# torognes/vsearch

Hardware: AMD Instinct MI355X
Metric: GCUPS (useful DP cells/s of the search16 global-alignment path: DP + traceback + CIGAR) (higher is better)
Workload: dtype int16

## Files before the change

include/vsx.h:

```cpp
#ifndef VSX_H
#define VSX_H

#include <stddef.h>
#include <stdint.h>

#ifdef __cplusplus
extern "C" {
#endif

#define VSX_API_VERSION 1000
#define VSX_SCORE_SENTINEL 32767

#define VSX_OK         0
#define VSX_EINVAL    -1
#define VSX_ENODEVICE -2
#define VSX_ENOMEM    -3
#define VSX_EHIP      -4

typedef struct vsx_ctx vsx_ctx;
typedef struct vsx_seqset vsx_seqset;
typedef struct vsx_plan vsx_plan;

typedef struct vsx_scoring {
  int64_t match;
  int64_t mismatch;
  int64_t gap_open_query_left;
  int64_t gap_open_target_left;
  int64_t gap_open_query_interior;
  int64_t gap_open_target_interior;
  int64_t gap_open_query_right;
  int64_t gap_open_target_right;
  int64_t gap_ext_query_left;
  int64_t gap_ext_target_left;
  int64_t gap_ext_query_interior;
  int64_t gap_ext_target_interior;
  int64_t gap_ext_query_right;
  int64_t gap_ext_target_right;
  int32_t n_mismatch;
} vsx_scoring;

typedef struct vsx_results {
  uint64_t   n_pairs;
  int16_t  * score;
  uint16_t * aligned;
  uint16_t * matches;
  uint16_t * mismatches;
  uint16_t * gaps;
  uint64_t * cigar_off;
  char     * cigar_blob;
  uint64_t   cigar_bytes;
  uint8_t  * verdict;
} vsx_results;

#define VSX_VERDICT_UNDECIDED 0
#define VSX_VERDICT_ACCEPTED  1
#define VSX_VERDICT_WEAK      2
#define VSX_VERDICT_REJECTED  3
typedef struct vsx_filter {
  int32_t iddef;
  int32_t leftjust, rightjust;
  int32_t pad;
  double  id, weak_id, maxid, mid, query_cov, target_cov;
  int64_t maxsubs, maxgaps, mincols, maxdiffs;
} vsx_filter;
int vsx_plan_set_filter(vsx_plan * plan, const vsx_filter * f);

typedef struct vsx_timing {
  float    forward_ms;
  float    traceback_ms;
  float    total_ms;
  uint32_t forward_launches;
  uint32_t traceback_launches;
  uint64_t cells;
  uint64_t dir_bytes;
} vsx_timing;

typedef struct vsx_plan_info {
  uint64_t tasks;
  uint64_t tasks_tilted;
  uint64_t tasks_tracked;
  uint32_t rows_dominant;
  uint32_t chunks;
  uint64_t tasks_max3;
  uint64_t tasks_sparse;
  uint64_t waves;
  uint64_t tasks_pair;
  uint64_t tasks_split;
} vsx_plan_info;

const char * vsx_version_string(void);
int vsx_device_count(void);
const char * vsx_last_error(void);

int vsx_create(vsx_ctx ** out, const vsx_scoring * scoring, int device);
void vsx_destroy(vsx_ctx * ctx);


int vsx_seqset_create(vsx_ctx * ctx, vsx_seqset ** out, uint64_t n,
                      const char * blob, uint64_t blob_bytes,
                      const uint64_t * offsets, const uint32_t * lengths);
int vsx_seqset_create_from_device(vsx_ctx * ctx, vsx_seqset ** out, uint64_t n,
                                  const void * d_blob, uint64_t blob_bytes,
                                  const uint64_t * offsets, const uint32_t * lengths);
int vsx_seqset_create_both_strands(vsx_ctx * ctx, vsx_seqset ** out, uint64_t n,
                                   const char * blob, uint64_t blob_bytes,
                                   const uint64_t * offsets, const uint32_t * lengths);
void vsx_seqset_destroy(vsx_seqset * s);
uint64_t vsx_seqset_count(const vsx_seqset * s);

int vsx_plan_create(vsx_ctx * ctx, vsx_plan ** out,
                    const vsx_seqset * queries, const vsx_seqset * targets,
                    uint64_t n_pairs, const uint32_t * qidx, const uint32_t * tidx,
                    uint64_t dir_budget_bytes);
int vsx_plan_run(vsx_plan * plan);
int vsx_plan_sync(vsx_plan * plan, vsx_timing * timing );
int vsx_plan_fetch(vsx_plan * plan, vsx_results * out);
int vsx_plan_describe(const vsx_plan * plan, vsx_plan_info * info);
#define VSX_HIT_RECORD_BYTES 24
int vsx_plan_export_hits(vsx_plan * plan, void * d_dst, uint64_t dst_bytes);
int vsx_plan_export_runs(vsx_plan * plan, void * d_dst, uint64_t dst_bytes, uint64_t * n_runs);
int64_t vsx_cigar_from_runs(const uint32_t * runs, uint32_t n, char * dst, uint64_t cap);
void vsx_plan_destroy(vsx_plan * plan);

int vsx_align_pairs_filtered(vsx_ctx * ctx, const vsx_seqset * queries, const vsx_seqset * targets,
                             uint64_t n_pairs, const uint32_t * qidx, const uint32_t * tidx,
                             const vsx_filter * filter, vsx_results * out);
int vsx_align_pairs(vsx_ctx * ctx, const vsx_seqset * queries, const vsx_seqset * targets,
// ... 27 lines not shown
```

vsearch_amd/_lib.py:

```python
import ctypes as C
import os

HERE = os.path.dirname(os.path.abspath(__file__))
LIB_PATH = os.environ.get("VSX_LIBRARY") or os.path.join(HERE, "libvsx.so")

VSX_OK, VSX_EINVAL, VSX_ENODEVICE, VSX_ENOMEM, VSX_EHIP = 0, -1, -2, -3, -4
SENTINEL = 32767

SYMBOLS = [
    "vsx_version_string", "vsx_device_count", "vsx_last_error", "vsx_create", "vsx_destroy",
    "vsx_seqset_create", "vsx_seqset_create_both_strands", "vsx_seqset_create_from_device", "vsx_seqset_destroy", "vsx_seqset_count",
    "vsx_plan_create", "vsx_plan_run", "vsx_plan_sync", "vsx_plan_fetch", "vsx_plan_export_hits", "vsx_plan_export_runs",
    "vsx_cigar_from_runs", "vsx_plan_destroy",
    "vsx_align_pairs", "vsx_align_pairs_filtered", "vsx_align_pairs_ranked", "vsx_ranked_free", "vsx_plan_set_filter", "vsx_results_free", "vsx_plan_describe",
]
EXACT_SYMBOLS = ["vsx_search_exact", "vsx_search_exact_last_stats", "vsx_internal_search_exact_host"]
SEARCH_SYMBOLS = ["vsx_search_opts_default", "vsx_searcher_create", "vsx_searcher_destroy", "vsx_searcher_db_text", "vsx_search_batch",
                  "vsx_search_batch_meta", "vsx_searcher_set_meta",
                  "vsx_hits_free", "vsx_search_candidates", "vsx_search_candidates_batch", "vsx_candidates_free", "vsx_lma_align", "vsx_allpairs_block", "vsx_allpairs_rows", "vsx_allpairs_stream", "vsx_cluster_fast", "vsx_cluster_out_free", "vsx_msa", "vsx_msa_out_free",
                  "vsx_msa_device", "vsx_msa_device_batch", "vsx_dust_mask", "vsx_abundance_ratio_cmp",
                  "vsx_multi_searcher_create", "vsx_multi_searcher_destroy", "vsx_multi_searcher_devices", "vsx_multi_searcher_replica",
                  "vsx_multi_search_batch", "vsx_multi_allpairs",
                  "vsx_chimera_opts_default", "vsx_uchime_ref", "vsx_chimera_last_stats",
                  "vsx_chimera_denovo_opts_default", "vsx_uchime_denovo", "vsx_chimera_denovo_last_stats",
# ... 294 lines not shown
class OrientResult(C.Structure):
    _fields_ = [("n_queries", C.c_uint64), ("n_fwd", C.c_uint64), ("n_rev", C.c_uint64), ("n_none", C.c_uint64),
                ("rec", C.POINTER(OrientRecord)), ("text", C.c_void_p), ("qual", C.c_void_p)]


class OrientStats(C.Structure):
    _fields_ = [(n, C.c_uint64) for n in ("queries_device", "queries_host_wordlength", "queries_host_qlen", "queries_host_forced")] + \
               [("queries_class", C.c_uint64 * ORIENT_CLASSES)] + \
               [(n, C.c_uint64) for n in ("windows", "words_distinct", "build_chunks", "build_keys")] + \
               [(n, C.c_double) for n in ("seconds_build", "seconds_stage", "seconds_count", "seconds_emit", "seconds_output",
                                          "seconds_total")]


class Scoring(C.Structure):
    _fields_ = [(n, C.c_int64) for n in (
        "match", "mismatch", "gap_open_query_left", "gap_open_target_left", "gap_open_query_interior",
        "gap_open_target_interior", "gap_open_query_right", "gap_open_target_right",
        "gap_ext_query_left", "gap_ext_target_left", "gap_ext_query_interior", "gap_ext_target_interior",
        "gap_ext_query_right", "gap_ext_target_right")] + [("n_mismatch", C.c_int32)]


class Results(C.Structure):
    _fields_ = [("n_pairs", C.c_uint64), ("score", C.POINTER(C.c_int16)), ("aligned", C.POINTER(C.c_uint16)),
                ("matches", C.POINTER(C.c_uint16)), ("mismatches", C.POINTER(C.c_uint16)),
                ("gaps", C.POINTER(C.c_uint16)), ("cigar_off", C.POINTER(C.c_uint64)),
                ("cigar_blob", C.POINTER(C.c_char)), ("cigar_bytes", C.c_uint64), ("verdict", C.POINTER(C.c_uint8))]


class Ranked(C.Structure):
    _fields_ = [("n_pairs", C.c_uint64), ("n_hits", C.c_uint64), ("pair", C.POINTER(C.c_uint32)), ("score", C.POINTER(C.c_int16)),
                ("aligned", C.POINTER(C.c_uint16)), ("matches", C.POINTER(C.c_uint16)), ("mismatches", C.POINTER(C.c_uint16)),
                ("gaps", C.POINTER(C.c_uint16)), ("verdict", C.POINTER(C.c_uint8)), ("id", C.POINTER(C.c_double)),
                ("cigar_off", C.POINTER(C.c_uint64)), ("cigar_blob", C.POINTER(C.c_char)), ("cigar_bytes", C.c_uint64),
                ("n_undecided", C.c_uint64), ("undecided", C.POINTER(C.c_uint32))]


class Filter(C.Structure):
    _fields_ = [("iddef", C.c_int32), ("leftjust", C.c_int32), ("rightjust", C.c_int32), ("pad", C.c_int32),
                ("id", C.c_double), ("weak_id", C.c_double), ("maxid", C.c_double), ("mid", C.c_double),
                ("query_cov", C.c_double), ("target_cov", C.c_double),
                ("maxsubs", C.c_int64), ("maxgaps", C.c_int64), ("mincols", C.c_int64), ("maxdiffs", C.c_int64)]


class PlanInfo(C.Structure):
    _fields_ = [("tasks", C.c_uint64), ("tasks_tilted", C.c_uint64), ("tasks_tracked", C.c_uint64),
                ("rows_dominant", C.c_uint32), ("chunks", C.c_uint32), ("tasks_max3", C.c_uint64),
                ("tasks_sparse", C.c_uint64), ("waves", C.c_uint64), ("tasks_pair", C.c_uint64),
                ("tasks_split", C.c_uint64)]


class Timing(C.Structure):
    _fields_ = [("forward_ms", C.c_float), ("traceback_ms", C.c_float), ("total_ms", C.c_float),
                ("forward_launches", C.c_uint32), ("traceback_launches", C.c_uint32),
                ("cells", C.c_uint64), ("dir_bytes", C.c_uint64)]


class ClusterOut(C.Structure):
    _fields_ = [("n", C.c_uint64), ("n_clusters", C.c_uint64), ("clusterno", C.POINTER(C.c_uint32)), ("hits", Hits)]


class MsaOut(C.Structure):
    _fields_ = [("alnlen", C.c_uint64), ("n_rows", C.c_uint64), ("conslen", C.c_uint64), ("rows", C.POINTER(C.c_char)),
                ("consensus", C.POINTER(C.c_char)), ("profile", C.POINTER(C.c_uint64))]


_lib = None


def load():
    global _lib
    if _lib is not None:
        return _lib
    if not os.path.exists(LIB_PATH):
        raise ImportError(
            f"{LIB_PATH} not found: build the HIP extension first (python -c 'import __graft_entry__ as g; "
            "g.build()' or make -C vsearch_amd/csrc). vsearch_amd has no CPU fallback.")
    lib = C.CDLL(LIB_PATH)
    vp = C.c_void_p
    lib.vsx_version_string.restype = C.c_char_p
    lib.vsx_last_error.restype = C.c_char_p
    lib.vsx_device_count.restype = C.c_int
    lib.vsx_create.argtypes = [C.POINTER(vp), C.POINTER(Scoring), C.c_int]
    lib.vsx_destroy.argtypes = [vp]
    lib.vsx_destroy.restype = None
    lib.vsx_seqset_create.argtypes = [vp, C.POINTER(vp), C.c_uint64, vp, C.c_uint64, vp, vp]
    lib.vsx_seqset_create_both_strands.argtypes = [vp, C.POINTER(vp), C.c_uint64, vp, C.c_uint64, vp, vp]
    lib.vsx_seqset_create_from_device.argtypes = [vp, C.POINTER(vp), C.c_uint64, vp, C.c_uint64, vp, vp]
    lib.vsx_seqset_destroy.argtypes = [vp]
    lib.vsx_seqset_destroy.restype = None
    lib.vsx_seqset_count.argtypes = [vp]
    lib.vsx_seqset_count.restype = C.c_uint64
    lib.vsx_plan_create.argtypes = [vp, C.POINTER(vp), vp, vp, C.c_uint64, vp, vp, C.c_uint64]
    lib.vsx_plan_run.argtypes = [vp]
    lib.vsx_plan_sync.argtypes = [vp, C.POINTER(Timing)]
    lib.vsx_plan_fetch.argtypes = [vp, C.POINTER(Results)]
    lib.vsx_plan_export_hits.argtypes = [vp, vp, C.c_uint64]
    lib.vsx_plan_export_runs.argtypes = [vp, vp, C.c_uint64, C.POINTER(C.c_uint64)]
    lib.vsx_cigar_from_runs.argtypes = [vp, C.c_uint32, vp, C.c_uint64]
    lib.vsx_cigar_from_runs.restype = C.c_int64
    lib.vsx_plan_destroy.argtypes = [vp]
    lib.vsx_plan_destroy.restype = None
    lib.vsx_plan_describe.argtypes = [vp, C.POINTER(PlanInfo)]
    lib.vsx_internal_settle_counts.argtypes = [vp, C.POINTER(C.c_uint64 * 2)]
    lib.vsx_internal_export_host.argtypes = [vp, vp, vp, C.c_uint64, C.POINTER(C.c_uint64)]
    lib.vsx_align_pairs.argtypes = [vp, vp, vp, C.c_uint64, vp, vp, C.POINTER(Results)]
    lib.vsx_align_pairs_filtered.argtypes = [vp, vp, vp, C.c_uint64, vp, vp, C.POINTER(Filter), C.POINTER(Results)]
    lib.vsx_align_pairs_ranked.argtypes = [vp, vp, vp, C.c_uint64, vp, vp, C.POINTER(Filter), C.c_int, C.POINTER(Ranked)]
# ... 140 lines not shown
```

vsearch_amd/csrc/vsx_device.hip:

```cpp
#include <hip/hip_runtime.h>
#include <type_traits>
#include <cstdlib>
#include <atomic>
#include "vsx_internal.h"

typedef unsigned int u32;
typedef unsigned int u32x4 __attribute__((ext_vector_type(4)));
typedef unsigned int u32x3 __attribute__((ext_vector_type(3)));
typedef short s2 __attribute__((ext_vector_type(2)));
typedef unsigned short us2 __attribute__((ext_vector_type(2)));

#define DEV __device__ __forceinline__
struct __attribute__((aligned(4))) Pair2 { unsigned int x, y; };

#define SIGN2 0x80008000u

DEV s2 S2(u32 x) { return __builtin_bit_cast(s2, x); }
DEV us2 U2(u32 x) { return __builtin_bit_cast(us2, x); }
DEV u32 UI(s2 x) { return __builtin_bit_cast(u32, x); }
DEV u32 UI(us2 x) { return __builtin_bit_cast(u32, x); }

DEV u32 sadd(u32 a, u32 b) { return UI(__builtin_elementwise_add_sat(S2(a), S2(b))); }
DEV u32 ssub(u32 a, u32 b) { return UI(__builtin_elementwise_sub_sat(S2(a), S2(b))); }
DEV u32 pmax(u32 a, u32 b) { return UI(__builtin_elementwise_max(S2(a), S2(b))); }
// ... 582 lines not shown
                  constexpr int NF = R + (R + 1) / 2;
                  constexpr int NFH = RT + (RT + 1) / 2, ZH = 4 * VSX_COLCK_NBH(RT);
                  auto flatc = [&](int z) -> u32 {
                    if (MIDCK)
                      {
                        const int hh = z / ZH, zz = z % ZH, r00 = hh * RT;
                        if (zz < RT) return hout[r00 + zz] + CK_REBIAS;
                        if (zz < NFH)
                          {
                            const int r0 = r00 + 2 * (zz - RT), r1 = (r0 + 1 < r00 + RT) ? r0 + 1 : r0;
                            return __builtin_amdgcn_perm(psubw(hout[r1], E[r1]), psubw(hout[r0], E[r0]), 0x06040200u);
                          }
                        return 0u;
                      }
                    if (z < R) return hout[z] + CK_REBIAS;
                    if (z < NF)
                      {
                        const int r0 = 2 * (z - R), r1 = r0 + 1 < R ? r0 + 1 : r0;
                        return __builtin_amdgcn_perm(psubw(hout[r1], E[r1]), psubw(hout[r0], E[r0]), 0x06040200u);
                      }
                    return 0u;
                  };
#pragma unroll
                  for (int z = 0; z < 4 * VSX_COLCK_NB(R, true); z += 4)
                    __builtin_nontemporal_store((u32x4) {flatc(z), flatc(z + 1), flatc(z + 2), flatc(z + 3)}, reinterpret_cast<u32x4 *>(cb + VSX_COLCK_CDW(VSX_COLCK_NB(R, true), ck_slot, z >> 2)));
                }
              else if (R % 2 == 0)
                {
                  auto flat = [&](int z) -> u32 { return z < R ? hout[z] : E[z - R]; };
#pragma unroll
                  for (int z = 0; z < 2 * R; z += 4)
                    __builtin_nontemporal_store((u32x4) {flat(z), flat(z + 1), flat(z + 2), flat(z + 3)}, reinterpret_cast<u32x4 *>(cb + VSX_COLCK_DW(R, lane, z >> 2)));
                }
              else
                {
                  u32 * cp = cb + lane * (2 * R);
#pragma unroll
                  for (int x = 0; x < R; ++x) { cp[x] = hout[x]; cp[R + x] = E[x]; }
                }
            }
          if (QPL) sym = symn;
      };
      int t_switch = 0;
      if (P.share_sub)
        {
          int dmin = 0x7fffffff;
          if (DA > 0 && DA < dmin) dmin = DA;
          if (DB > 0 && DB < dmin) dmin = DB;
#pragma unroll
          for (int m = 32; m >= 1; m >>= 1) { const int o = __shfl_xor(dmin, m, 64); dmin = o < dmin ? o : dmin; }
          t_switch = __builtin_amdgcn_readfirstlane(dmin == 0x7fffffff ? 0 : dmin - 1) & ~1;
          if (t_switch > steps) t_switch = steps & ~1;
        }
      int t = 0;
      qrt = qrt_i_pk; rt = pack16(P.rt_i);
      for (; t < t_switch && (TRACK || t < 16); t += 2)
        {
          step(t, hprev, hnext, profA, profB, std::true_type {}, std::false_type {}, std::false_type {});
          step(t + 1, hnext, hprev, profB, profA, std::true_type {}, std::true_type {}, std::false_type {});
        }
      if (!TRACK)
        {
          const u32 lpk = (u32) l * 0x00010001u;
          lv1 = psubw(lv1, psubw(0u, lpk));
          for (; t + 32 <= t_switch; t += 16)
            {
              const int tb = t & ~15;
#pragma unroll
              for (int k = 0; k < 16; k += 2)
                {
                  step(tb + k, hprev, hnext, profA, profB, std::true_type {}, std::false_type {}, std::integral_constant<int, 2> {});
                  step(tb + k + 1, hnext, hprev, profB, profA, std::true_type {}, std::true_type {}, std::integral_constant<int, 2> {});
                }
            }
          for (; t < t_switch; t += 2)
            {
              step(t, hprev, hnext, profA, profB, std::true_type {}, std::false_type {}, std::true_type {});
              step(t + 1, hnext, hprev, profB, profA, std::true_type {}, std::true_type {}, std::true_type {});
            }
          lv1 = psubw(lv1, lpk);
        }
      for (; t < steps; t += 2)
        {
          step(t, hprev, hnext, profA, profB, std::false_type {}, std::false_type {}, std::false_type {});
          step(t + 1, hnext, hprev, profB, profA, std::false_type {}, std::true_type {}, std::false_type {});
        }

      if (s + 1 < nstrips)
        {
          __builtin_amdgcn_fence(__ATOMIC_RELEASE, "agent");
          __builtin_amdgcn_fence(__ATOMIC_ACQUIRE, "agent");
        }
    }

#pragma unroll
  for (int m = 8; m >= 1; m >>= 1)
    {
      hmin = pmin(hmin, (u32) __shfl_xor((int) hmin, m, 16));
      hmax = pmax(hmax, (u32) __shfl_xor((int) hmax, m, 16));
    }
  const int l_last = (total_lanes - 1) & 15;
  score = (u32) __shfl((int) score, l_last, 16);
  leave = (u32) __shfl((int) leave, l_last, 16);
  if (l == 0)
    {
      const int mnA = (int16_t) (hmin & 0xffff), mnB = (int16_t) (hmin >> 16);
      const int mxA = (int16_t) (hmax & 0xffff), mxB = (int16_t) (hmax >> 16);
      VsxSlotOut oA, oB;
      score = psubw(score, BIAS);
      oA.score = (int16_t) ((int) (int16_t) (score & 0xffff) - (DA > 0 ? (Q + DA - 2) * tl : 0));
      oB.score = (int16_t) ((int) (int16_t) (score >> 16) - (DB > 0 ? (Q + DB - 2) * tl : 0));
      oA.leave = (uint16_t) (leave & 0xffff); oB.leave = (uint16_t) (leave >> 16); oA.pad = 0; oB.pad = 0;
      oA.overflow = (mnA <= P.smin || mxA >= 32767) ? 1 : 0;
      oB.overflow = (mnB <= P.smin || mxB >= 32767) ? 1 : 0;
      if (sub_on)
        {
          slot_out[(size_t) tix * VSX_TASK_SLOTS + 2 * g] = oA;
          slot_out[(size_t) tix * VSX_TASK_SLOTS + 2 * g + 1] = oB;
        }
    }
}

DEV u32 half_lo(u32 w, bool hi) { return hi ? (w >> 16) : w; }
DEV int wave_max_i32(int v)
{
#pragma unroll
  for (int m = 32; m >= 1; m >>= 1) { const int o = __shfl_xor(v, m, 64); v = o > v ? o : v; }
  return v;
}

DEV void rank_note(const VsxFilterDev & FL, u32 pid, u32 verdict, int score, double idv)
{
  if (FL.rank_counts == nullptr) return;
// ... 1340 lines not shown
```

vsearch_amd/csrc/vsx_host.cpp:

```cpp
#include "../../include/vsx.h"
#include "vsx_internal.h"
#include "vsx_private.h"

#include <hip/hip_runtime.h>
#include <algorithm>
#include <cinttypes>
#include <cstdio>
#include <cstdlib>
#include <cstring>
#include <sched.h>
#include <thread>
#include <atomic>
#include <condition_variable>
#include <mutex>
#include <chrono>
#include <deque>
#include <functional>
#include <memory>
#include <numeric>
#include <string>
#include <vector>

using vsxp::fail;
using vsxp::DevBuf;
// ... 616 lines not shown
          vsx_launch_max3_selftest(d_bad.p, c->stream) == hipSuccess &&
          hipMemcpyAsync(bad2, d_bad.p, 8, hipMemcpyDeviceToHost, c->stream) == hipSuccess && hipStreamSynchronize(c->stream) == hipSuccess)
        {
          const uint32_t bad = bad2[0];
          if (bad) std::fprintf(stderr, "libvsx: device %d: v_pk_maximum3_f16 disagrees with the integer maximum on %u probes -- MAX3 class disabled\n", device, bad);
          g_max3_state[device].store(bad ? 2 : 1);
          if (bad2[1])
            {
              std::fprintf(stderr, "libvsx: device %d: v_perm_b32 sign selectors disagree on %u probes -- the first traceback kernel is used\n", device, bad2[1]);
              vsx_internal_set_tb_v2(device, 0);
            }
        }
      else
        {
          (void) hipGetLastError();
          std::fprintf(stderr, "libvsx: device %d: the MAX3 / v_perm_b32 self-test could not run -- MAX3 class and second traceback kernel disabled\n", device);
          g_max3_state[device].store(2);
          vsx_internal_set_tb_v2(device, 0);
        }
    }
  else if (device >= 64) vsx_internal_set_tb_v2(device, 0);

  if (geqi == geti && geti > 0 && P.share_sub && !c->tb_packed && !c->force_fallback &&
      std::min(match, mism) + 2 * geti >= 0 && 2 * geti - geql >= 0 &&
      std::max(match, mism) + 2 * geti <= 255 && 2 * geti - geql <= 255 &&
      geti <= 127 && std::max({goqi, goti, goqr + geqr - geti, gotr + getr - geti, goql + geql + goqi}) <= 127 &&
      !(std::getenv("VSX_TILT") && std::strcmp(std::getenv("VSX_TILT"), "0") == 0))
    {
      const int g = geti;
      VsxDevParams & T = c->Pt;
      T = P;
      T.tilt = g;
      T.qrq_i_pk = pk(goqi + geqi - g); T.rq_i_pk = pk(geqi - g);
      T.qrq_r_pk = pk(goqr + geqr - g); T.rq_r_pk = pk(geqr - g);
      T.qrt_i = goti + geti - g; T.rt_i = geti - g;
      T.qrt_r = gotr + getr - g; T.rt_r = getr - g;
      std::vector<int16_t> htop_t(VSX_TABLE_LEN), hleft_t(VSX_TABLE_LEN), matrix_t(256);
      for (int j = 0; j < VSX_TABLE_LEN; ++j)
        {
          htop_t[j] = (int16_t) sat16((int) htop[j] + (j - 1) * g);
          hleft_t[j] = (int16_t) sat16((int) hleft[j] + (j - 1) * g);
        }
      for (int x = 0; x < 256; ++x) matrix_t[x] = (int16_t) sat16(matrix[x] + 2 * g);
      if ((e = c->d_htop_t.alloc(VSX_TABLE_LEN)) != hipSuccess || (e = c->d_hleft_t.alloc(VSX_TABLE_LEN)) != hipSuccess ||
          (e = c->d_matrix_t.alloc(256)) != hipSuccess ||
          (e = hipMemcpy(c->d_htop_t.p, htop_t.data(), VSX_TABLE_LEN * 2, hipMemcpyHostToDevice)) != hipSuccess ||
          (e = hipMemcpy(c->d_hleft_t.p, hleft_t.data(), VSX_TABLE_LEN * 2, hipMemcpyHostToDevice)) != hipSuccess ||
          (e = hipMemcpy(c->d_matrix_t.p, matrix_t.data(), 512, hipMemcpyHostToDevice)) != hipSuccess)
        {
          cleanup();
          return fail(VSX_EHIP, "vsx_create: %s", hipGetErrorString(e));
        }
      T.htop = c->d_htop_t.p; T.hleft = c->d_hleft_t.p; T.matrix = c->d_matrix_t.p;
    }
  { std::lock_guard<std::mutex> lk(g_ctx_mu); g_ctxs.push_back(c); }
  *out = c;
  return VSX_OK;
}

void vsx_destroy(vsx_ctx * c)
{
  if (!c) return;
  { std::lock_guard<std::mutex> lk(g_ctx_mu); g_ctxs.erase(std::remove(g_ctxs.begin(), g_ctxs.end(), c), g_ctxs.end()); }
  (void) hipSetDevice(c->device);
  if (c->stream) { (void) hipStreamSynchronize(c->stream); (void) hipStreamDestroy(c->stream); }
  if (c->stream2) { (void) hipStreamSynchronize(c->stream2); (void) hipStreamDestroy(c->stream2); }
  if (c->stream_b) { (void) hipStreamSynchronize(c->stream_b); (void) hipStreamDestroy(c->stream_b); }
  if (c->stream_up) { (void) hipStreamSynchronize(c->stream_up); (void) hipStreamDestroy(c->stream_up); }
  if (c->stream_dn) { (void) hipStreamSynchronize(c->stream_dn); (void) hipStreamDestroy(c->stream_dn); }
  c->shared_dir[0].reset();
  c->shared_dir[1].reset();
  c->shared_dir[2].reset();
  c->shared_slab.reset();
  c->pool.retire();
  delete c;
}

static int seqset_common(vsx_ctx * ctx, vsx_seqset ** out, uint64_t n, const void * blob, bool blob_on_device,
                         uint64_t blob_bytes, const uint64_t * offsets, const uint32_t * lengths, bool both_strands = false,
                         int case_bits = 0 )
{
  if (!ctx || !out || (n && (!offsets || !lengths)) || (blob_bytes && !blob))
    return fail(VSX_EINVAL, "vsx_seqset_create: null argument");
  *out = nullptr;
  for (uint64_t i = 0; i < n; ++i)
    if (offsets[i] + lengths[i] > blob_bytes)
      return fail(VSX_EINVAL, "vsx_seqset_create: sequence %" PRIu64 " exceeds the blob", i);
  VSX_HIP(hipSetDevice(ctx->device));
  auto * s = new vsx_seqset;
  s->ctx = ctx;
  s->device = ctx->device;
  s->n = n;
  s->bytes = blob_bytes;
  s->off.assign(offsets, offsets + n);
  s->len.assign(lengths, lengths + n);
  uint64_t code_bytes = blob_bytes;
  if (both_strands)
    {
      s->n = 2 * n;
      s->off.resize(2 * n);
      s->len.resize(2 * n);
      for (uint64_t k = 0; k < n; ++k) { s->off[n + k] = code_bytes; s->len[n + k] = lengths[k]; code_bytes += lengths[k]; }
      s->bytes = code_bytes;
    }
  hipError_t e = hipSuccess;
  ScratchPool * pl = (code_bytes <= VSX_SEQSET_POOLED_BYTES) ? &ctx->pool : nullptr;
// ... 562 lines not shown
      cur.strip_elems += strip;
      pl->dir_bytes_total += dwords * 4;
      if (cur.launches.empty() || cur.launches.back().rows != pt.rows ||
          cur.launches.back().track != pt.track || cur.launches.back().tilt != pt.tilt || cur.launches.back().nq != pt.nq)
        cur.launches.push_back(Launch {pt.rows, pt.track, pt.tilt, pt.nq, (uint32_t) x, 0, cur.pair_first + cur.pair_count, 0});
      cur.launches.back().count++;
      if (strip != 0) cur.launches.back().multi = true;
      cur.launches.back().pair_count += pt.n;
      t_pair0[x] = np_out;
      np_out += pt.n;
      const uint64_t slab = t_slab[x];
      t_slab[x] = cur.slab_words;
      cur.slab_words += slab;
      cur.pair_count += pt.n;
      cur.task_count++;
    }
  run_threads(ntt, [&](int th) {
    const size_t lo = NT * (size_t) th / (size_t) ntt, hi = NT * (size_t) (th + 1) / (size_t) ntt;
    for (size_t x = lo; x < hi; ++x)
      {
        const ProtoTask & pt = protos[x];
        const VsxTask & t = pl->tasks[x];
        uint64_t slab = t_slab[x];
        for (uint32_t sl = 0; sl < pt.n; ++sl)
          {
            const size_t o = (size_t) t_pair0[x] + sl;
            pl->pair_slot[o] = (uint32_t) x * VSX_TASK_SLOTS + sl;
            pl->pair_ids[o] = pt.pair[sl];
            pl->slab_off[o] = slab;
            slab += (uint64_t) t.qlen + t.tlen[sl] + 1;
          }
      }
  });
  close_chunk();
  const double tc3 = now();

  uint64_t max_dir = 1, max_strip = 1, max_slab = 1, worst_runs = 0;
  for (const Chunk & c : pl->chunks)
    {
      max_dir = std::max(max_dir, c.dir_dwords + VSX_CK_SLACK_DW);
      max_strip = std::max(max_strip, c.strip_elems);
      max_slab = std::max(max_slab, c.slab_words);
      worst_runs += c.slab_words;
    }
  const size_t ngp = pl->pair_ids.size();
  pl->runs_capacity = std::min<uint64_t>(worst_runs, std::max<uint64_t>(16ull << 20, 48ull * ngp)) + 1;
  if (const char * c = std::getenv("VSX_TEST_RUNS_CAP")) pl->runs_capacity = std::min<uint64_t>(pl->runs_capacity, std::max<uint64_t>(1, std::strtoull(c, nullptr, 10)));
  VSX_HIP(pl->d_tasks.alloc(&ctx->pool, pl->tasks.size()));
  VSX_HIP(pl->d_pair_slot.alloc(&ctx->pool, ngp));
  VSX_HIP(pl->d_pair_ids.alloc(&ctx->pool, ngp));
  VSX_HIP(pl->d_slab_off.alloc(&ctx->pool, ngp));
  VSX_HIP(pl->d_slot.alloc(&ctx->pool, pl->tasks.size() * VSX_TASK_SLOTS));
  VSX_HIP(pl->d_out.alloc(&ctx->pool, n_pairs));
  VSX_HIP(pl->d_cursor.alloc(&ctx->pool, 2));
  {
    const uint64_t np = std::max<uint64_t>(n_pairs, 1);
    const uint64_t width[7] = {2, 2, 2, 2, 2, 1, 8};
    uint64_t at = 0;
    for (int x = 0; x < 7; ++x) { pl->soa_off[x] = at; at += (np * width[x] + 15) & ~15ull; }
    pl->soa_bytes = at;
    VSX_HIP(pl->d_soa.alloc(&ctx->pool, at));
    uint8_t * b = pl->d_soa.p;
    pl->soa.score = reinterpret_cast<int16_t *>(b + pl->soa_off[0]);
    pl->soa.aligned = reinterpret_cast<uint16_t *>(b + pl->soa_off[1]);
    pl->soa.matches = reinterpret_cast<uint16_t *>(b + pl->soa_off[2]);
    pl->soa.mismatches = reinterpret_cast<uint16_t *>(b + pl->soa_off[3]);
    pl->soa.gaps = reinterpret_cast<uint16_t *>(b + pl->soa_off[4]);
    pl->soa.verdict = b + pl->soa_off[5];
    pl->soa.text_off = reinterpret_cast<uint64_t *>(b + pl->soa_off[6]);
  }
  {
    std::lock_guard<std::mutex> lk(ctx->stage_mu);
    if (!ctx->cursor_slots.empty()) { pl->h_cursor = ctx->cursor_slots.back(); ctx->cursor_slots.pop_back(); }
  }
  if (!pl->h_cursor) VSX_HIP(hipHostMalloc(reinterpret_cast<void **>(&pl->h_cursor), 64, hipHostMallocDefault));
  for (int k = 0; k < 2; ++k)
    {
      const uint64_t need = (k == 0 ? max_dir : max_slab) * 4;
      uint64_t seen = ctx->req_hwm[k].load();
      while (need > seen && !ctx->req_hwm[k].compare_exchange_weak(seen, need)) { }
    }
  VSX_HIP(pl->d_dir[0].alloc(ctx->shared_dir[pl->dir_slot], &ctx->pool, max_dir));
  VSX_HIP(pl->d_strip.alloc(&ctx->pool, max_strip));
  VSX_HIP(pl->d_slab.alloc(ctx->shared_slab, &ctx->pool, max_slab));
  VSX_HIP(pl->d_runs.alloc(&ctx->pool, pl->runs_capacity));
  pl->text_capacity = std::min<uint64_t>(6 * worst_runs + 8 * (uint64_t) ngp, std::max<uint64_t>(32ull << 20, 128ull * ngp)) + 16;
  if (const char * c = std::getenv("VSX_TEST_TEXT_CAP")) pl->text_capacity = std::min<uint64_t>(pl->text_capacity, std::max<uint64_t>(4, std::strtoull(c, nullptr, 10)));
  VSX_HIP(pl->d_text.alloc(&ctx->pool, pl->text_capacity));
  if (!pl->tasks.empty())
    VSX_HIP(hipMemcpyAsync(pl->d_tasks.p, pl->tasks.data(), pl->tasks.size() * sizeof(VsxTask), hipMemcpyHostToDevice, ctx->stream_up));
  if (ngp)
    {
      VSX_HIP(hipMemcpyAsync(pl->d_pair_slot.p, pl->pair_slot.data(), ngp * 4, hipMemcpyHostToDevice, ctx->stream_up));
      VSX_HIP(hipMemcpyAsync(pl->d_pair_ids.p, pl->pair_ids.data(), ngp * 4, hipMemcpyHostToDevice, ctx->stream_up));
      VSX_HIP(hipMemcpyAsync(pl->d_slab_off.p, pl->slab_off.data(), ngp * 8, hipMemcpyHostToDevice, ctx->stream_up));
    }
  VSX_HIP(hipEventCreate(&pl->ev_begin));
  VSX_HIP(hipEventCreate(&pl->ev_end));
  for (Chunk & c : pl->chunks)
    {
      VSX_HIP(hipEventCreate(&c.e0));
      VSX_HIP(hipEventCreate(&c.e1));
      VSX_HIP(hipEventCreate(&c.e1b));
      VSX_HIP(hipEventCreate(&c.e2));
    }
  VSX_HIP(hipStreamSynchronize(ctx->stream_up));
  if (timing)
    std::fprintf(stderr, "vsx_plan_create: %llu pairs, %zu tasks: classify %.2f ms, group %.2f ms (budget query %.2f), tasks %.2f ms, device buffers + upload %.2f ms\n",
                 (unsigned long long) n_pairs, pl->tasks.size(), (tc1 - tc0) * 1e3, (tc2 - tc1) * 1e3, t_budget * 1e3, (tc3 - tc2) * 1e3, (now() - tc3) * 1e3);
  *out = pl.release();
  return VSX_OK;
}

int vsx_plan_set_filter(vsx_plan * pl, const vsx_filter * f)
{
  if (!pl) return fail(VSX_EINVAL, "vsx_plan_set_filter: null plan");
  pl->filter = VsxFilterDev {};
  if (!f) return VSX_OK;
  if (f->iddef < 0 || f->iddef > 4) return fail(VSX_EINVAL, "vsx_plan_set_filter: iddef must be 0..4");
  VsxFilterDev & d = pl->filter;
  d.enabled = 1; d.iddef = f->iddef; d.leftjust = f->leftjust; d.rightjust = f->rightjust;
  d.id = f->id; d.weak_id = f->weak_id; d.maxid = f->maxid; d.mid = f->mid; d.query_cov = f->query_cov; d.target_cov = f->target_cov;
  d.maxsubs = f->maxsubs; d.maxgaps = f->maxgaps; d.mincols = f->mincols; d.maxdiffs = f->maxdiffs;
  pl->ran = false;
  return VSX_OK;
}

static int plan_set_ranked(vsx_plan * pl)
{
  if (!pl->filter.enabled) return VSX_OK;
  vsx_ctx * ctx = pl->ctx;
  const size_t n = (size_t) pl->n_pairs;
  VSX_HIP(hipSetDevice(ctx->device));
  VSX_HIP(pl->d_rank_counts.alloc(&ctx->pool, 2));
  VSX_HIP(pl->d_kept_pair.alloc(&ctx->pool, n + 1));
  VSX_HIP(pl->d_kept_id.alloc(&ctx->pool, n + 1));
  VSX_HIP(pl->d_refused_pair.alloc(&ctx->pool, n + 1));
  pl->filter.rank_counts = pl->d_rank_counts.p;
  pl->filter.kept_pair = pl->d_kept_pair.p;
  pl->filter.kept_id = pl->d_kept_id.p;
  pl->filter.refused_pair = pl->d_refused_pair.p;
  return VSX_OK;
}

int vsx_plan_run(vsx_plan * pl)
{
  if (!pl) return fail(VSX_EINVAL, "vsx_plan_run: null plan");
  vsx_ctx * ctx = pl->ctx;
  VSX_HIP(hipSetDevice(ctx->device));
  hipStream_t st = pl->alt_fwd ? ctx->stream_b : ctx->stream, st2 = ctx->stream2;
  const int slot = pl->dir_slot;
  VSX_HIP(hipMemsetAsync(pl->d_cursor.p, 0, 2 * sizeof(unsigned long long), st));
  if (pl->filter.rank_counts) VSX_HIP(hipMemsetAsync(pl->d_rank_counts.p, 0, 2 * sizeof(uint32_t), st));
  VSX_HIP(hipEventRecord(pl->ev_begin, st));
  for (size_t k = 0; k < pl->chunks.size(); ++k)
    {
      Chunk & c = pl->chunks[k];
      uint32_t * dir = pl->d_dir[0].p;
      if (k >= 1) VSX_HIP(hipStreamWaitEvent(st, pl->chunks[k - 1].e2, 0));
      else if (ctx->ev_tb_used[slot]) VSX_HIP(hipStreamWaitEvent(st, ctx->ev_tb[slot], 0));
      VSX_HIP(hipEventRecord(c.e0, st));
      for (const Launch & L : c.launches)
        {
          VsxDevParams Pf = L.tilt ? ctx->Pt : ctx->P;
          Pf.max3 = (L.tilt == 2) ? 1 : 0;
          static const bool one_off = std::getenv("VSX_ONESTRIP") && std::strcmp(std::getenv("VSX_ONESTRIP"), "0") == 0;
          VSX_HIP(vsx_launch_forward(L.rows, L.track, L.nq, (L.multi || (one_off && L.nq < 8)) ? 0 : 1, Pf, pl->d_tasks.p + L.first, L.count,
                                    pl->Q->codes(), pl->T->codes(), dir, pl->d_strip.p,
                                    pl->d_slot.p + (size_t) L.first * VSX_TASK_SLOTS, st));
        }
      VSX_HIP(hipEventRecord(c.e1, st));
      VSX_HIP(hipStreamWaitEvent(st2, c.e1, 0));
      VSX_HIP(hipEventRecord(c.e1b, st2));
      for (size_t li = 0; li < c.launches.size();)
        {
          const Launch & L = c.launches[li];
          uint32_t pair_count = L.pair_count;
          size_t lj = li + 1;
          while (lj < c.launches.size() && c.launches[lj].rows == L.rows &&
                 c.launches[lj].track == L.track && c.launches[lj].tilt == L.tilt) { pair_count += c.launches[lj].pair_count; ++lj; }
          VsxDevParams Pb = L.tilt ? ctx->Pt : ctx->P;
          Pb.max3 = (L.tilt == 2) ? 1 : 0;
          VSX_HIP(vsx_launch_traceback_ck(L.rows, L.track == 0 ? 1 : 0, Pb, pl->filter, pl->d_tasks.p, pl->d_pair_slot.p + L.pair_first,
                                         pl->d_pair_ids.p + L.pair_first, pair_count, pl->Q->codes(), pl->T->codes(),
                                         dir, pl->d_slot.p, pl->d_slab.p, pl->d_slab_off.p + L.pair_first,
                                         pl->d_runs.p, pl->runs_capacity, pl->d_cursor.p, pl->d_out.p, st2));
          li = lj;
        }
      VSX_HIP(hipEventRecord(c.e2, st2));
    }
  if (pl->chunks.empty()) VSX_HIP(hipStreamWaitEvent(st2, pl->ev_begin, 0));
  VSX_HIP(hipEventRecord(ctx->ev_tb[slot], st2));
  ctx->ev_tb_used[slot] = true;
  VSX_HIP(vsx_launch_cigar_text(pl->d_out.p, pl->d_pair_ids.p, (uint32_t) pl->pair_ids.size(), pl->d_runs.p, pl->runs_capacity,
                               pl->d_text.p, pl->text_capacity, pl->d_cursor.p + 1, pl->soa, st2));
  VSX_HIP(hipMemcpyAsync(pl->h_cursor, pl->d_cursor.p, 2 * sizeof(unsigned long long), hipMemcpyDeviceToHost, st2));
  VSX_HIP(hipEventRecord(pl->ev_end, st2));
  pl->ran = true;
  pl->host_patched = false;
  return VSX_OK;
}

int vsx_plan_sync(vsx_plan * pl, vsx_timing * tm)
{
  if (!pl) return fail(VSX_EINVAL, "vsx_plan_sync: null plan");
  if (!pl->ran) return fail(VSX_EINVAL, "vsx_plan_sync: plan has not been run");
  VSX_HIP(hipSetDevice(pl->ctx->device));
  VSX_HIP(hipEventSynchronize(pl->ev_end));
  if (tm)
    {
      *tm = vsx_timing {};
      for (Chunk & c : pl->chunks)
        {
          float a = 0, b = 0;
          VSX_HIP(hipEventElapsedTime(&a, c.e0, c.e1));
          VSX_HIP(hipEventElapsedTime(&b, c.e1b, c.e2));
          tm->forward_ms += a;
          tm->traceback_ms += b;
          tm->forward_launches += (uint32_t) c.launches.size();
          tm->traceback_launches += 1;
        }
      VSX_HIP(hipEventElapsedTime(&tm->total_ms, pl->ev_begin, pl->ev_end));
      tm->cells = pl->cells;
      tm->dir_bytes = pl->dir_bytes_total;
    }
  return VSX_OK;
}

int vsx_plan_describe(const vsx_plan * pl, vsx_plan_info * info)
{
  if (!pl || !info) return fail(VSX_EINVAL, "vsx_plan_describe: null argument");
  *info = vsx_plan_info {};
  info->tasks = pl->tasks.size();
  info->chunks = (uint32_t) pl->chunks.size();
  uint64_t best = 0;
  for (const Chunk & c : pl->chunks)
    for (const Launch & L : c.launches)
      {
        if (L.nq == 2 || L.nq == 4) info->tasks_sparse += L.count;
        if (L.nq == 8) info->tasks_pair += L.count;
        if (L.nq == 16) info->tasks_split += L.count;
        info->waves += (L.nq == 2 || L.nq == 4) ? (L.count + (uint32_t) L.nq - 1) / (uint32_t) L.nq : L.count;
        if (L.tilt) info->tasks_tilted += L.count;
        if (L.tilt == 2) info->tasks_max3 += L.count;
        if (L.track) info->tasks_tracked += L.count;
        if (L.count > best) { best = L.count; info->rows_dominant = (uint32_t) L.rows; }
      }
  return VSX_OK;
}

static void append_cigar(std::string & s, const uint32_t * runs, uint32_t n)
{
  static const char ops[4] = {'M', 'I', 'D', '?'};
  char buf[16];
  for (uint32_t k = n; k-- > 0;)
    {
      const uint32_t len = runs[k] >> 2;
      if (len > 1) { int w = snprintf(buf, sizeof buf, "%u", len); s.append(buf, (size_t) w); }
      s.push_back(ops[runs[k] & 3]);
    }
}

struct FetchDest {
  int16_t * score; uint16_t * aligned, * matches, * mismatches, * gaps; uint64_t * cigar_off; uint8_t * verdict;
  char ** blob; uint64_t * blob_used;
};

static int settle_runs(vsx_plan * pl, unsigned long long & used, unsigned long long & text_used)
{
  vsx_ctx * ctx = pl->ctx;
  if (!pl->ran) { int rc = vsx_plan_run(pl); if (rc != VSX_OK) return rc; }
  int rc = vsx_plan_sync(pl, nullptr);
  if (rc != VSX_OK) return rc;
  VSX_HIP(hipSetDevice(ctx->device));
  used = pl->h_cursor[0]; text_used = pl->h_cursor[1];
  if (used > pl->runs_capacity)
    {
// ... 554 lines not shown
```

vsearch_amd/csrc/vsx_internal.h:

```cpp
#ifndef VSX_INTERNAL_H
#define VSX_INTERNAL_H

#include <stdint.h>
#include <hip/hip_runtime_api.h>

#define VSX_TASK_SLOTS 8
#define VSX_GROUP_LANES 16
#define VSX_MAX_SEQLEN_SUM 65535LL
#define VSX_MAX_SEQLEN_PRODUCT 25000000LL
#define VSX_TABLE_LEN (65536 + 64)
#define VSX_CODE_SLACK 64
#define VSX_CK_SLACK_DW 4096
#ifndef VSX_MID_MIN_ROWS
#define VSX_MID_MIN_ROWS 18
#endif
#define VSX_MID(R_, TILT_) ((TILT_) && (R_) >= VSX_MID_MIN_ROWS)
#define VSX_SPLIT_ROWS(R_) ((R_) == 10 || (R_) == 16)

struct VsxDevParams {
  uint32_t match_pk;
  uint32_t qrq_i_pk, rq_i_pk;
  uint32_t qrq_r_pk, rq_r_pk;
  int32_t  qrt_i, rt_i;
  int32_t  qrt_r, rt_r;
  int32_t  match, mismatch;
  int32_t  smin;
  int32_t  n_mismatch;
  int32_t  share_sub;
  int32_t  top_open, top_step;
  int32_t  tilt;
  int32_t  max3;
  const int16_t * htop;
  const int16_t * hleft;
  const int16_t * matrix;
};

struct VsxTask {
  uint64_t qoff;
  uint64_t toff[VSX_TASK_SLOTS];
  uint64_t dir_off;
  uint64_t strip_off;
  uint32_t tlen[VSX_TASK_SLOTS];
  uint32_t qlen;
  uint32_t steps;
  uint32_t rows;
  uint32_t group0;
};

struct VsxFilterDev {
  int32_t enabled, iddef, leftjust, rightjust;
  double  id, weak_id, maxid, mid, query_cov, target_cov;
  int64_t maxsubs, maxgaps, mincols, maxdiffs;
  uint32_t * rank_counts;
  uint32_t * kept_pair;
  double   * kept_id;
  uint32_t * refused_pair;
};

struct VsxSlotOut {
  int16_t  score;
  uint16_t overflow;
  uint16_t leave;
  uint16_t pad;
};

struct VsxPairOut {
  int16_t  score;
  uint16_t aligned, matches, mismatches, gaps;
  uint16_t pad;
  uint32_t nruns;
  uint64_t run_off;
};

struct VsxSoaOut {
  int16_t  * score;
  uint16_t * aligned, * matches, * mismatches, * gaps;
  uint8_t  * verdict;
  uint64_t * text_off;
};

struct VsxRankedOut {
  uint32_t * pair;
  int16_t  * score;
  uint16_t * aligned, * matches, * mismatches, * gaps;
// ... 114 lines not shown
```

Baseline: 8413.

## Add provably-safe early termination to tilted max3 forward DP sweep

Adds an early-stop check inside the tilted single-query max3 forward loop. Every few 16-step blocks it computes upper bounds on the score any remaining path can still reach and compares them against lower bounds from the current end-of-column values. When the remaining steps provably cannot change the result, it writes the final score, sets the leave mask and exits the loop. This targets wasted DP steps on long targets, at the cost of extra bound computation, cross-lane permutes and readlanes during the sweep. It also adds a skipped-steps counter exposed through the timing struct, plus profiling scripts.

```diff
diff --git a/include/vsx.h b/include/vsx.h
--- a/include/vsx.h
+++ b/include/vsx.h
@@ -73,6 +73,7 @@
   uint32_t traceback_launches;
   uint64_t cells;
   uint64_t dir_bytes;
+  uint64_t steps_skipped;
 } vsx_timing;
 
 typedef struct vsx_plan_info {
diff --git a/profiles/early_stop/predict.py b/profiles/early_stop/predict.py
--- /dev/null
+++ b/profiles/early_stop/predict.py
@@ -0,0 +1,56 @@
+#!/usr/bin/env python3
+import os
+import sys
+
+import numpy as np
+
+ROOT = os.path.dirname(os.path.dirname(os.path.dirname(os.path.abspath(__file__))))
+sys.path.insert(0, ROOT)
+
+from tests import test_early_stop_math as M
+from vsearch_amd import workload
+
+
+def main():
+    nq = int(sys.argv[1]) if len(sys.argv) > 1 else 24
+    qlen = int(sys.argv[2]) if len(sys.argv) > 2 else 250
+    tlen = int(sys.argv[3]) if len(sys.argv) > 3 else 1000
+    R = 16 if qlen > 160 else 10
+    db, off, ln, fam = workload.make_family_db(2000, tlen, device="cpu")
+    qa, qoff, qln, src = workload.make_queries(db, off, ln, nq, qlen, device="cpu")
+    qi, ti = workload.family_candidates(src, fam)
+    db, qa = bytes(db.numpy()).decode(), bytes(qa.numpy()).decode()
+    s = M.DEFAULT
+    total = skipped = fired = 0
+    scores = []
+    for k in range(nq):
+        q = qa[int(qoff[k]):int(qoff[k]) + int(qln[k])]
+        ts = [db[int(off[x]):int(off[x]) + int(ln[x])] for x in ti[qi == k]]
+        Q = len(q)
+        sch = M.Schedule(Q, R)
+        dmin, dmax = min(map(len, ts)), max(map(len, ts))
+        steps = ((dmax + 3) & ~3) + 16
+        t_switch = (dmin - 1) & ~1
+        per = []
+        for t in ts:
+            H, En, htop, score, leave, margin, lv1s = M._dp(q, t, s)
+            scores.append(score)
+            per.append((M._plain_tables(sch, H, htop, s), H, En, htop, len(t)))
+        t_exit = None
+        t_ = (Q + 15) & ~15
+        while t_ + 32 <= t_switch:
+            if all(M._plain_criterion(sch, tabs, H, En, htop, D, s, t_ - 1)[0] for tabs, H, En, htop, D in per):
+                t_exit = t_
+                break
+            t_ += 16
+        total += steps
+        if t_exit is not None:
+            skipped += steps - t_exit
+            fired += 1
+        print(f"task {k}: Q {Q} D {dmin}..{dmax} steps {steps} exit {t_exit}", flush=True)
+    print(f"tasks {nq}, exits {fired}, steps {total}, skipped {skipped} = {100.0 * skipped / total:.1f} %, "
+          f"scores min/median/max {min(scores)}/{int(np.median(scores))}/{max(scores)}")
+
+
+if __name__ == "__main__":
+    main()
diff --git a/profiles/early_stop/skipped.py b/profiles/early_stop/skipped.py
--- /dev/null
+++ b/profiles/early_stop/skipped.py
@@ -0,0 +1,38 @@
+#!/usr/bin/env python3
+import os
+import sys
+
+import numpy as np
+import torch
+
+ROOT = os.path.dirname(os.path.dirname(os.path.dirname(os.path.abspath(__file__))))
+sys.path.insert(0, ROOT)
+
+from vsearch_amd import Aligner, SequenceSet, workload
+
+
+def main():
+    qlen = int(sys.argv[1]) if len(sys.argv) > 1 else 250
+    dlen = int(sys.argv[2]) if len(sys.argv) > 2 else 1000
+    dbn = int(sys.argv[3]) if len(sys.argv) > 3 else 1_000_000
+    nq, cands = 100_000, 8
+    dev = torch.device("cuda", 0)
+    db_ascii, db_off, db_len, fam = workload.make_family_db(dbn, dlen, seed=17, device=dev)
+    q_ascii, q_off, q_len, src = workload.make_queries(db_ascii, db_off, db_len, nq, qlen, seed=11, device=dev)
+    qidx, tidx = workload.family_candidates(src, fam, per_query=cands, seed=5)
+    with Aligner(device=0) as al:
+        T = SequenceSet(al, blob=db_ascii.numel(), offsets=db_off, lengths=db_len, device_ptr=db_ascii.data_ptr())
+        Q = SequenceSet(al, blob=q_ascii.numel(), offsets=q_off, lengths=q_len, device_ptr=q_ascii.data_ptr())
+        plan = al.plan(Q, T, qidx, tidx)
+        info = plan.describe()
+        plan.run()
+        tm = plan.sync()
+        plan.close()
+    dmax = db_len[tidx].reshape(nq, cands).max(axis=1).astype(np.int64)
+    steps = int((((dmax + 3) & ~3) + 16).sum())
+    print(f"{qlen} x {dlen}: tasks {info['tasks']} (split {info['tasks_split']}, max3 {info['tasks_max3']}), steps {steps}, "
+          f"skipped {int(tm.steps_skipped)} = {100.0 * tm.steps_skipped / steps:.2f} %, forward {tm.forward_ms:.3f} ms")
+
+
+if __name__ == "__main__":
+    main()
diff --git a/vsearch_amd/_lib.py b/vsearch_amd/_lib.py
--- a/vsearch_amd/_lib.py
+++ b/vsearch_amd/_lib.py
@@ -370,7 +370,7 @@
 class Timing(C.Structure):
     _fields_ = [("forward_ms", C.c_float), ("traceback_ms", C.c_float), ("total_ms", C.c_float),
                 ("forward_launches", C.c_uint32), ("traceback_launches", C.c_uint32),
-                ("cells", C.c_uint64), ("dir_bytes", C.c_uint64)]
+                ("cells", C.c_uint64), ("dir_bytes", C.c_uint64), ("steps_skipped", C.c_uint64)]
 
 
 class ClusterOut(C.Structure):
diff --git a/vsearch_amd/csrc/vsx_device.hip b/vsearch_amd/csrc/vsx_device.hip
--- a/vsearch_amd/csrc/vsx_device.hip
+++ b/vsearch_amd/csrc/vsx_device.hip
@@ -658,6 +658,63 @@
           t_switch = __builtin_amdgcn_readfirstlane(dmin == 0x7fffffff ? 0 : dmin - 1) & ~1;
           if (t_switch > steps) t_switch = steps & ~1;
         }
+      constexpr bool EARLY = TILT && MAX3 && ONE && NQ == 1 && !PAIR && !TRACK && R >= 4;
+      bool es_fired = false;
+      const int da_ = DA, db_ = DB;
+      auto early_check = [&](const int tn) __attribute__((always_inline)) -> int {
+        if constexpr (EARLY)
+          {
+            int ln = lane, DA = da_, DB = db_;
+            asm volatile("" : "+v"(ln), "+v"(DA), "+v"(DB));
+            const int l = ln & 15;
+            const int t1 = tn - 1, ll = total_lanes - 1, c = t1 - ll;
+            const int W0 = P.es_w0, e = P.es_e, W1 = W0 + tl, W2 = tl - e, rr = P.es_rr;
+            const u32 el = (u32) __builtin_amdgcn_ds_bpermute((ln - l + ll) << 2, (int) E[R - 1]);
+            const int eA = (int) (el & 0xffffu), eB = (int) (el >> 16);
+            const int lbA = eA - tl * (c + 1) - (DA - 2 - c) * rr, lbB = eB - tl * (c + 1) - (DB - 2 - c) * rr;
+            const int top = (int) P.htop[t1] + (int) BIAS16;
+            {
+              const int a1 = top + W1 * Q - tl * t1, a2 = top + W2 * Q - tl * t1;
+              const int cA = DA - 1 - t1, cB = DB - 1 - t1;
+              const int uA = a1 - e * cA < a2 + W0 * cA ? a1 - e * cA : a2 + W0 * cA;
+              const int uB = a1 - e * cB < a2 + W0 * cB ? a1 - e * cB : a2 + W0 * cB;
+              const int dA = DA > 0 ? uA - lbA : -1, dB = DB > 0 ? uB - lbB : -1;
+              int d = dA > dB ? dA : dB;
+              const int d1 = __builtin_amdgcn_readlane(d, 16), d2 = __builtin_amdgcn_readlane(d, 32), d3 = __builtin_amdgcn_readlane(d, 48);
+              d = __builtin_amdgcn_readlane(d, 0);
+              d = d > d1 ? d : d1; d = d > d2 ? d : d2; d = d > d3 ? d : d3;
+              if (d >= 0) { const int w = (d / P.es_rate) & ~15; return w < 16 ? 16 : w; }
+            }
+            const u32 w1pk = pack16(W1), w2pk = pack16(W2);
+            u32 m1 = hprev[0], m2 = hprev[0];
+#pragma unroll
+            for (int r = 1; r < R - 1; ++r) { m1 = pmaxu(m1 + w1pk, hprev[r]); m2 = pmaxu(m2 + w2pk, hprev[r]); }
+            m1 += w1pk; m2 += w2pk;
+            if (l < ll)
+              {
+                m1 = pmaxu(pmaxu(m1, hprev[R - 1]), hnext[R - 1] + pack16(tl - e));
+                m2 = pmaxu(pmaxu(m2, hprev[R - 1]), hnext[R - 1] + pack16(tl + W0));
+              }
+            if (l == 0)
+              {
+                m1 = pmaxu(m1, pack16(top + W1 * rc0));
+                m2 = pmaxu(m2, pack16(top + W2 * rc0));
+              }
+            const int j = t1 - l, rb = (ll - l) * R;
+            const int b1 = W1 * rb - tl * j, b2 = W2 * rb - tl * j;
+            const int cA = DA - 1 - j, cB = DB - 1 - j;
+            const int f1A = (int) (m1 & 0xffffu) + b1 - e * cA, f2A = (int) (m2 & 0xffffu) + b2 + W0 * cA;
+            const int f1B = (int) (m1 >> 16) + b1 - e * cB, f2B = (int) (m2 >> 16) + b2 + W0 * cB;
+            const bool okA = DA == 0 || (f1A < f2A ? f1A : f2A) < lbA;
+            const bool okB = DB == 0 || (f1B < f2B ? f1B : f2B) < lbB;
+            if (!__all((l > ll) || (okA && okB))) return 16;
+            const int sA = DA > 0 ? eA - (DA - 2 - c) * (rr - tl) : 0, sB = DB > 0 ? eB - (DB - 2 - c) * (rr - tl) : 0;
+            score = ((u32) sA & 0xffffu) | ((u32) sB << 16);
+            if (ln == 0 && P.es_skipped != nullptr) atomicAdd(P.es_skipped, (unsigned long long) (steps - tn));
+            return 0;
+          }
+        return 16;
+      };
       int t = 0;
       qrt = qrt_i_pk; rt = pack16(P.rt_i);
       for (; t < t_switch && (TRACK || t < 16); t += 2)
@@ -669,8 +726,18 @@
         {
           const u32 lpk = (u32) l * 0x00010001u;
           lv1 = psubw(lv1, psubw(0u, lpk));
+          int es_next = (EARLY && P.es_on) ? ((Q + 15) & ~15) : 0x7fffffff;
           for (; t + 32 <= t_switch; t += 16)
             {
+              if constexpr (EARLY)
+                {
+                  if (__builtin_expect(t >= es_next, 0))
+                    {
+                      const int w = early_check(t);
+                      if (w == 0) { es_fired = true; t = steps; break; }
+                      es_next = t + w;
+                    }
+                }
               const int tb = t & ~15;
 #pragma unroll
               for (int k = 0; k < 16; k += 2)
@@ -685,6 +752,7 @@
               step(t + 1, hnext, hprev, profB, profA, std::true_type {}, std::true_type {}, std::true_type {});
             }
           lv1 = psubw(lv1, lpk);
+          if constexpr (EARLY) { if (es_fired) leave = lv1 & ((DA > 0 ? 0x0000ffffu : 0u) | (DB > 0 ? 0xffff0000u : 0u)); }
         }
       for (; t < steps; t += 2)
         {
diff --git a/vsearch_amd/csrc/vsx_host.cpp b/vsearch_amd/csrc/vsx_host.cpp
--- a/vsearch_amd/csrc/vsx_host.cpp
+++ b/vsearch_amd/csrc/vsx_host.cpp
@@ -692,6 +692,17 @@
           return fail(VSX_EHIP, "vsx_create: %s", hipGetErrorString(e));
         }
       T.htop = c->d_htop_t.p; T.hleft = c->d_hleft_t.p; T.matrix = c->d_matrix_t.p;
+      {
+        bool ok = true;
+        for (int k = 0; k < 12; ++k) ok = ok && c->pen[k] >= 0;
+        const int e_min = std::min({geql, getl, geqi, geti, geqr, getr});
+        const int w0 = std::max({match, mism, 0}) + e_min;
+        if (ok && 32 * (w0 + g) <= 0xFFFF - 0x7BFF)
+          {
+            T.es_on = 1; T.es_w0 = w0; T.es_e = e_min; T.es_rr = geqr;
+            T.es_rate = std::max(1, w0 + geql);
+          }
+      }
     }
   { std::lock_guard<std::mutex> lk(g_ctx_mu); g_ctxs.push_back(c); }
   *out = c;
@@ -1360,7 +1371,7 @@
   VSX_HIP(pl->d_slab_off.alloc(&ctx->pool, ngp));
   VSX_HIP(pl->d_slot.alloc(&ctx->pool, pl->tasks.size() * VSX_TASK_SLOTS));
   VSX_HIP(pl->d_out.alloc(&ctx->pool, n_pairs));
-  VSX_HIP(pl->d_cursor.alloc(&ctx->pool, 2));
+  VSX_HIP(pl->d_cursor.alloc(&ctx->pool, 3));
   {
     const uint64_t np = std::max<uint64_t>(n_pairs, 1);
     const uint64_t width[7] = {2, 2, 2, 2, 2, 1, 8};
@@ -1458,7 +1469,7 @@
   VSX_HIP(hipSetDevice(ctx->device));
   hipStream_t st = pl->alt_fwd ? ctx->stream_b : ctx->stream, st2 = ctx->stream2;
   const int slot = pl->dir_slot;
-  VSX_HIP(hipMemsetAsync(pl->d_cursor.p, 0, 2 * sizeof(unsigned long long), st));
+  VSX_HIP(hipMemsetAsync(pl->d_cursor.p, 0, 3 * sizeof(unsigned long long), st));
   if (pl->filter.rank_counts) VSX_HIP(hipMemsetAsync(pl->d_rank_counts.p, 0, 2 * sizeof(uint32_t), st));
   VSX_HIP(hipEventRecord(pl->ev_begin, st));
   for (size_t k = 0; k < pl->chunks.size(); ++k)
@@ -1472,6 +1483,7 @@
         {
           VsxDevParams Pf = L.tilt ? ctx->Pt : ctx->P;
           Pf.max3 = (L.tilt == 2) ? 1 : 0;
+          Pf.es_skipped = pl->d_cursor.p + 2;
           static const bool one_off = std::getenv("VSX_ONESTRIP") && std::strcmp(std::getenv("VSX_ONESTRIP"), "0") == 0;
           VSX_HIP(vsx_launch_forward(L.rows, L.track, L.nq, (L.multi || (one_off && L.nq < 8)) ? 0 : 1, Pf, pl->d_tasks.p + L.first, L.count,
                                     pl->Q->codes(), pl->T->codes(), dir, pl->d_strip.p,
@@ -1502,7 +1514,7 @@
   ctx->ev_tb_used[slot] = true;
   VSX_HIP(vsx_launch_cigar_text(pl->d_out.p, pl->d_pair_ids.p, (uint32_t) pl->pair_ids.size(), pl->d_runs.p, pl->runs_capacity,
                                pl->d_text.p, pl->text_capacity, pl->d_cursor.p + 1, pl->soa, st2));
-  VSX_HIP(hipMemcpyAsync(pl->h_cursor, pl->d_cursor.p, 2 * sizeof(unsigned long long), hipMemcpyDeviceToHost, st2));
+  VSX_HIP(hipMemcpyAsync(pl->h_cursor, pl->d_cursor.p, 3 * sizeof(unsigned long long), hipMemcpyDeviceToHost, st2));
   VSX_HIP(hipEventRecord(pl->ev_end, st2));
   pl->ran = true;
   pl->host_patched = false;
@@ -1531,6 +1543,7 @@
       VSX_HIP(hipEventElapsedTime(&tm->total_ms, pl->ev_begin, pl->ev_end));
       tm->cells = pl->cells;
       tm->dir_bytes = pl->dir_bytes_total;
+      tm->steps_skipped = pl->h_cursor[2];
     }
   return VSX_OK;
 }
diff --git a/vsearch_amd/csrc/vsx_internal.h b/vsearch_amd/csrc/vsx_internal.h
--- a/vsearch_amd/csrc/vsx_internal.h
+++ b/vsearch_amd/csrc/vsx_internal.h
@@ -30,6 +30,8 @@
   int32_t  top_open, top_step;
   int32_t  tilt;
   int32_t  max3;
+  int32_t  es_on, es_w0, es_e, es_rr, es_rate;
+  unsigned long long * es_skipped;
   const int16_t * htop;
   const int16_t * hleft;
   const int16_t * matrix;
```

New measurement: 9470, median of 6. 12.6% higher.
